# databricks/spark-sklearn

Hardware: NVIDIA H100
Metric: candidate-fits/sec (higher is better)
Workload: dtype f64

## Files before the change

include/b200gs.h:

```cpp
#ifndef B200GS_H
#define B200GS_H

#include <stdint.h>

#ifdef __cplusplus
extern "C" {
#endif

typedef struct gs_handle gs_handle;

enum gs_status {
    GS_OK = 0,
    GS_ERR_CUDA = -1,
    GS_ERR_ARG = -2,
    GS_ERR_NO_DATA = -3,
    GS_ERR_UNSUPPORTED = -4,
    GS_ERR_NUMERIC = -5
};

enum gs_kernel { GS_KERNEL_LINEAR = 0, GS_KERNEL_RBF = 1, GS_KERNEL_POLY = 2, GS_KERNEL_SIGMOID = 3 };
enum gs_dtype { GS_F32 = 0, GS_F64 = 1 };

enum gs_flags {
    GS_RETURN_TRAIN = 1,
// ... 105 lines not shown
    int32_t *test_block, *train_block;
    float *shift;
    float *block_shift;
    double *ystat;
    double *G;
    double *T, *Tw;
    float *A;
    float *rhs;
    double *means;
    float *coef;
    double *qk, *qt;
    double *scores;
    int32_t *n_iter;
    double *gap;
} gs_linear_debug;
int gs_debug_linear(gs_handle *h, int32_t mode, int32_t n_cand, const double *alpha, const double *l1_ratio, int32_t fit_intercept,
                    double tol, int32_t max_iter, int32_t refit, gs_linear_debug *out);

int gs_debug_gemm_nt(gs_handle *h, const float *A, int32_t M, const float *B, int32_t N, int32_t K, float *C);
int gs_debug_gemm_f64(gs_handle *h, const double *A, int32_t M, const double *B, int32_t N, int32_t K, double *C);

double gs_svc_predicted_iterations(int32_t kernel, double C, double gamma, int32_t d);
int32_t gs_svc_cluster_count(const double *cost_desc, int32_t n, int32_t sm_count);
void gs_svc_schedule(const double *cost_desc, int32_t n, int32_t sm_count, int32_t *n_cluster, int32_t *n_exclusive);

typedef struct gs_profile {
    float ms_total;
    float ms_h2d;
    float ms_gram;
    float ms_kernel_matrix;
    float ms_solve;
    float ms_score;
    int64_t launches;
    int64_t smo_iterations;
    double solve_bytes;
    double gram_flops;
    double gram_bytes;
    int64_t h2d_bytes;
    int64_t d2h_bytes;
    float ms_tensor;
    double tensor_flops;
} gs_profile;
int gs_get_profile(const gs_handle *h, gs_profile *out);

#ifdef __cplusplus
}
// ... 3 lines not shown
```

spark_sklearn_b200/csrc/api.cu:

```cuda
#include "common.cuh"
#include <algorithm>
#include <cmath>
#include <cstring>
#include <cstdio>
#include <cstdlib>
#include <map>
#include <numeric>

static std::string g_create_error;

double gs_score_from_counts(int kind, int pos_class, int n_classes, const int *cnt)
{
    auto sup = [&](int c) { return (double)cnt[c * 3 + 0]; };
    auto tp = [&](int c) { return (double)cnt[c * 3 + 1]; };
    auto prd = [&](int c) { return (double)cnt[c * 3 + 2]; };
    auto f1c = [&](int c) { const double den = sup(c) + prd(c); return den > 0 ? 2.0 * tp(c) / den : 0.0; };
    double n = 0, correct = 0;
    for (int c = 0; c < n_classes; c++) { n += sup(c); correct += tp(c); }
    if (!(n > 0)) return NAN;
    switch (kind) {
    case GS_SCORE_DEFAULT: return correct / n;
    case GS_SCORE_BALANCED_ACCURACY: {
        double s = 0; int k = 0;
        for (int c = 0; c < n_classes; c++) if (sup(c) > 0) { s += tp(c) / sup(c); k++; }
// ... 281 lines not shown
{
    if (kernel != GS_KERNEL_RBF) return C;
    const double gd = gamma * (double)d;
    if (!(gd > 0)) return C;
    return std::min(4.0 + 10.3 * std::pow(C * gd, 0.95), 9.0 + 7.3 / gd);
}

extern "C" int32_t gs_svc_cluster_count(const double *cost_desc, int32_t n, int32_t sm_count)
{
    if (!cost_desc || n < 2 || sm_count < 4) return 0;
    double total = 0;
    for (int q = 0; q < n; q++) total += cost_desc[q];
    const int nmax = std::min(n - 1, sm_count / 4);
    double best = 0, clustered = 0;
    int pick = 0;
    for (int k = 0; k <= nmax; k++) {
        const double f = std::max({(total + clustered) / sm_count, 0.9 * cost_desc[k], k > 0 ? 0.5 * cost_desc[0] : 0.0});
        if (k == 0 || f < 0.97 * best) { best = f; pick = k; }
        clustered += cost_desc[k];
    }
    return pick;
}

extern "C" void gs_svc_schedule(const double *cost_desc, int32_t n, int32_t sm_count, int32_t *n_cluster, int32_t *n_exclusive)
{
    if (n_cluster) *n_cluster = 0;
    if (n_exclusive) *n_exclusive = 0;
    if (!cost_desc || n < 2 || sm_count < 8) return;
    std::vector<double> suffix(n + 1, 0.0);
    for (int q = n - 1; q >= 0; q--) suffix[q] = suffix[q + 1] + cost_desc[q];
    double best = -1;
    int bc = 0, be = 0;
    const int max_cl = std::min(n - 1, sm_count / 4);
    for (int nc = 0; nc <= max_cl; nc++) {
        for (int ne = 0; nc + ne < n && 4 * nc + ne <= sm_count - 8; ne++) {
            const int left = sm_count - 4 * nc - ne;
            double t = std::max(0.50 * suffix[nc + ne] / left, 0.78 * cost_desc[nc + ne]);
            if (nc > 0) t = std::max(t, 0.34 * cost_desc[0]);
            if (ne > 0) t = std::max(t, 0.52 * cost_desc[nc]);
            if (best < 0 || t < 0.97 * best || (t < best && nc + ne <= bc + be)) { best = t; bc = nc; be = ne; }
        }
    }
    if (n_cluster) *n_cluster = bc;
    if (n_exclusive) *n_exclusive = be;
}

static int svc_run(gs_handle *h, int n_cand, const int32_t *kernel, const double *Cv, const double *gamma,
                   double tol, int max_iter, uint32_t flags, bool refit, bool nu,
                   double *test_scores, double *train_scores, int32_t *n_iter, int32_t *n_sv,
                   float *fit_ms, float *score_ms, double *pair_coef, double *rho_out, int32_t *pair_iter)
{
    const char *who = nu ? "gs_nusvc" : "gs_svc";
    if (!h) return GS_ERR_ARG;
    if (h->n == 0) { gs_set_error(h, std::string(who) + ": no dataset (call gs_set_data first)"); return GS_ERR_NO_DATA; }
    if (!h->classification) { gs_set_error(h, std::string(who) + ": dataset has no class labels"); return GS_ERR_ARG; }
    if (h->n_classes < 2 || h->n_classes > 32) { gs_set_error(h, std::string(who) + ": need 2..32 classes"); return GS_ERR_UNSUPPORTED; }
    if (n_cand <= 0 || !kernel || !Cv || !gamma) { gs_set_error(h, std::string(who) + ": bad arguments"); return GS_ERR_ARG; }
    if (!h->sample_w.empty()) {
        gs_set_error(h, std::string(who) + ": sample weights (a C per row) are not supported by the SMO kernels; class weights are (gs_set_class_weight)");
        return GS_ERR_UNSUPPORTED;
    }
    if (h->class_w_sets > 1 && h->class_w_sets != (refit ? 1 : h->n_splits)) {
        gs_set_error(h, std::string(who) + ": gs_set_class_weight was given a weight set per split, but not for this number of splits"); return GS_ERR_ARG;
    }
    GS_CUDA(cudaSetDevice(h->device));
    cudaStream_t st = h->stream;
    const int n = (int)h->n, d = (int)h->d, nc = h->n_classes;
// ... 199 lines not shown
        int max_slots = 0;
        bool lean_ok = lmax < 16383 && !(getenv("B200GS_SMO_LEAN") && atoi(getenv("B200GS_SMO_LEAN")) == 0);
        for (int q = 0; q < np && lean_ok; q++) {
            lean_ok = probs[q].nseg > 0 && probs[q].nslots <= smo_lean_max_slots();
            max_slots = std::max(max_slots, probs[q].nslots);
        }
        auto launch_single = [&](const int *ord, int cnt, cudaStream_t s_, bool exclusive) -> cudaError_t {
            for (int inst = search.fast ? 1 : 0; inst >= 0; inst--) {
                const cudaError_t e = lean_ok ? launch_smo_lean(d_probs, ord, cnt, max_slots, inst == 1, exclusive, s_)
                                              : launch_smo(d_probs, ord, cnt, lmax, inst == 1, (int)ldk, s_, &why);
                if (e != cudaSuccess) return e;
                pf.launches++;
            }
            return cudaSuccess;
        };
        int cl = 0, n_cl = 0, n_ex = 0;
        if (!nu && lmax > 2048) {
            if (np * 8 <= h->sm_count) { cl = 8; n_cl = np; }
            else if (np * 4 <= h->sm_count) { cl = 4; n_cl = np; }
            else if (np * 2 <= h->sm_count) { cl = 2; n_cl = np; }
            else {
                std::vector<double> sorted_cost(np);
                for (int q = 0; q < np; q++) sorted_cost[q] = cost[order[q]];
                if (lean_ok) gs_svc_schedule(sorted_cost.data(), np, h->sm_count, &n_cl, &n_ex);
                else n_cl = gs_svc_cluster_count(sorted_cost.data(), np, h->sm_count);
                if (n_cl > 0) cl = 4;
            }
        }
        if (const char *e = getenv("B200GS_SMO_CLUSTER")) { cl = atoi(e); if (n_cl == 0) n_cl = std::max(1, np * 6 / 100); }
        if (const char *e = getenv("B200GS_SMO_CLUSTER_N")) n_cl = std::min(np, atoi(e));
        if (!(cl == 2 || cl == 4 || cl == 8) || lmax > smo_colown_max_rows(cl) || lmax <= 2048) n_cl = 0;
        n_ex = std::max(0, std::min(n_ex, np - n_cl));
        if (nu) {
            for (int inst = search.fast ? 1 : 0; inst >= 0; inst--) {
                const cudaError_t ce = launch_smo_nu(d_probs, nullptr, d_nu, d_order, np, lmax, inst == 1, st, &why);
                if (ce != cudaSuccess) { gs_set_error(h, why.empty() ? std::string("launch_smo_nu: ") + cudaGetErrorString(ce) : why); return why.empty() ? GS_ERR_CUDA : GS_ERR_UNSUPPORTED; }
                pf.launches++;
            }
        } else if (n_cl > 0 || n_ex > 0) {
            cudaEvent_t ready = h->evp.get();
            cudaEventRecord(ready, st);
            cudaError_t ce = cudaSuccess;
            if (n_cl > 0) {
                for (int inst = search.fast ? 1 : 0; inst >= 0 && ce == cudaSuccess; inst--) {
                    ce = launch_smo_colown(d_probs, d_order, n_cl, lmax, cl, inst == 1, st);
                    pf.launches++;
                }
                if (ce != cudaSuccess) { gs_set_error(h, std::string("launch_smo_colown: ") + cudaGetErrorString(ce)); return GS_ERR_CUDA; }
            }
// ... 60 lines not shown
        for (int q = 0; q < np; q++) {
            const int t = prob_task[q];
            task_iter[t] += info[(size_t)q * 4]; task_sv[t] += info[(size_t)q * 4 + 2];
            task_fit_ms[t] += (double)(ns[(size_t)q * 12 + 1] - ns[(size_t)q * 12]) * 1e-6;
            total_iter += info[(size_t)q * 4];
            solve_bytes += (double)info[(size_t)q * 4] * 2.0 * probs[q].l * 4.0;
            if (!std::isfinite(rho[q])) { if (refit) { gs_set_error(h, std::string(who) + "_refit: non-finite intercept"); return GS_ERR_NUMERIC; } task_bad[t] = 1; }
        }
        if (getenv("B200GS_SMO_TIMELINE") && atoi(getenv("B200GS_SMO_TIMELINE"))) {
            unsigned long long t0 = ~0ull;
            for (int q = 0; q < np; q++) if (ns[(size_t)q * 12]) t0 = std::min(t0, ns[(size_t)q * 12]);
            auto span = [&](int a, int b, const char *name) {
                if (b <= a) return;
                double s0 = 1e30, s1 = 0, e0 = 1e30, e1 = 0; long long it_max = 0;
                for (int i = a; i < b; i++) {
                    const int q = order[i];
                    const double st_ = (double)(ns[(size_t)q * 12] - t0) * 1e-6, en = (double)(ns[(size_t)q * 12 + 1] - t0) * 1e-6;
                    s0 = std::min(s0, st_); s1 = std::max(s1, st_); e0 = std::min(e0, en); e1 = std::max(e1, en);
                    it_max = std::max<long long>(it_max, info[(size_t)q * 4]);
                }
                fprintf(stderr, "[timeline] %-9s %4d problems: starts %.2f..%.2f ms, ends %.2f..%.2f ms, longest %lld iterations\n",
                        name, b - a, s0, s1, e0, e1, it_max);
            };
            span(0, n_cl, "cluster"); span(n_cl, n_cl + n_ex, "exclusive"); span(n_cl + n_ex, np, "shared");
            for (int i = 0; i < std::min(np, 16); i++) {
                const int q = order[i];
                fprintf(stderr, "[timeline]   #%d: %d iterations, %.2f -> %.2f ms (%.3f us/iteration)\n", i, info[(size_t)q * 4],
                        (double)(ns[(size_t)q * 12] - t0) * 1e-6, (double)(ns[(size_t)q * 12 + 1] - t0) * 1e-6,
                        (double)(ns[(size_t)q * 12 + 1] - ns[(size_t)q * 12]) * 1e-3 / std::max(1, info[(size_t)q * 4]));
            }
        }
        if (getenv("B200GS_SMO_PROF") && atoi(getenv("B200GS_SMO_PROF"))) {
            int qmax = 0;
            for (int q = 1; q < np; q++) if (info[(size_t)q * 4] > info[(size_t)qmax * 4]) qmax = q;
            const unsigned long long *pn = &ns[(size_t)qmax * 12];
            const double it = (double)info[(size_t)qmax * 4];
            fprintf(stderr, "[smo prof] longest problem: %d iters, %.1f ms (%.2f us/iter); cycles/iter by slot:", info[(size_t)qmax * 4],
                    (double)(pn[1] - pn[0]) * 1e-6, (double)(pn[1] - pn[0]) * 1e-3 / it);
            for (int e = 0; e < 10; e++) fprintf(stderr, " %.0f", pn[2 + e] / it);
            fprintf(stderr, "\n");
        }
        for (size_t v = 0; v < vtasks.size(); v++)
            for (int e = 0; e < 4; e++) all_counts[(size_t)vtask_id[v] * 4 + e] = counts[v * 4 + e];
        if (!refit && h->score_kind == GS_SCORE_ROC_AUC) {
            for (size_t v = 0; v < vtasks.size(); v++) {
                const int k = vtasks[v].fold;
                double na_te = 0, nb_te = 0, na_tr = 0, nb_tr = 0;
                for (int r = 0; r < n; r++) {
                    const bool b = r >= h->class_start[1];
                    if (h->is_test(r, k)) (b ? nb_te : na_te) += 1;
                    else if (h->is_train(r, k)) (b ? nb_tr : na_tr) += 1;
                }
                const unsigned long long *a = &score_raw[v * 4];
                task_score[(size_t)vtask_id[v] * 2 + 0] = na_te * nb_te > 0 ? ((double)a[0] + 0.5 * (double)a[1]) / (na_te * nb_te) : NAN;
                task_score[(size_t)vtask_id[v] * 2 + 1] = na_tr * nb_tr > 0 ? ((double)a[2] + 0.5 * (double)a[3]) / (na_tr * nb_tr) : NAN;
            }
        } else if (!refit && h->score_kind != GS_SCORE_DEFAULT) {
            for (size_t v = 0; v < vtasks.size(); v++)
                for (int sp = 0; sp < 2; sp++)
                    task_score[(size_t)vtask_id[v] * 2 + sp] =
                        gs_score_from_counts(h->score_kind, h->score_pos, nc, &class_counts[(v * 2 + sp) * nc * 3]);
        }
        if (refit) {
// ... 252 lines not shown
```

spark_sklearn_b200/csrc/smo_lean.cu:

```cuda
#include "smo_common.cuh"
#include <algorithm>
#include <type_traits>

namespace {

using namespace smo;

constexpr unsigned LF_UP = 4u, LF_LOW = 8u;
constexpr int POS_SHIFT = 18, SLOT_SHIFT = 4;
constexpr unsigned SLOT_MASK = 0x3fffu;
constexpr unsigned PF_INERT = 0xfffffff0u;

__device__ __forceinline__ unsigned lean_flags(bool ypos, int st)
{
    const bool up = ypos ? st != ST_UPPER : st != ST_LOWER;
    const bool low = ypos ? st != ST_LOWER : st != ST_UPPER;
    return (unsigned)st | (up ? LF_UP : 0u) | (low ? LF_LOW : 0u);
}

template <int N, int I = 0, class F>
__device__ __forceinline__ void lean_loop(F &&f)
{
    if constexpr (I < N) { f(std::integral_constant<int, I>{}); lean_loop<N, I + 1>(f); }
}
// ... 52 lines not shown
                 "mad.wide.u32 wi, %4, 0x20000000, 0x3800000000000000;\n\t"
                 "mad.wide.u32 wj, %5, 0x20000000, 0x3800000000000000;\n\t"
                 "mov.b64 fi, wi;\n\t"
                 "mov.b64 fj, wj;\n\t"
                 "mul.rn.f64 fi, fi, %6;\n\t"
                 "mul.rn.f64 fj, fj, %7;\n\t"
                 "add.rn.f64 fi, fi, fj;\n\t"
                 "add.rn.f64 %0, %0, fi;\n\t"
                 "and.b32 t, %8, %9;\n\t"
                 "setp.ne.u32 pu, t, 0;\n\t"
                 "setp.gt.and.f64 pb, %0, %1, pu;\n\t"
                 "setp.eq.and.f64 pe, %0, %1, pu;\n\t"
                 "selp.f64 %1, %0, %1, pb;\n\t"
                 "selp.b32 %2, %10, %2, pb;\n\t"
                 "selp.b32 %3, 1, %3, pe;\n\t"
                 "}"
                 : "+d"(m), "+d"(la), "+r"(la_k), "+r"(tie)
                 : "r"(__float_as_uint(kvi)), "r"(__float_as_uint(kvj)), "d"(a), "d"(b), "r"(fm), "n"(1u << (2 * K)), "n"(K));
}

struct LeanRed {
    unsigned a_hi[32], a_lo[32], a_pf[32];
    unsigned b_k1[32], b_pf[32], b_k2[32], b_fl[32];
    float b_kq[32]; double b_al[32], b_mg[32];
    double al_i;
    double bc_d[4]; int bc_i[2];
    unsigned x_hi[32], x_lo[32], x_pf[32];
    float x_kq[32]; double x_al[32], x_mg[32];
    double dm[32], dm2[32]; int cnt[32];
    int seg_slot[5], seg_col[4];
    int ysplit;
};

template <int NT, int G, bool FAST, bool PROF>
__global__ void __launch_bounds__(NT, (NT * G >= 4096 || NT >= 1024 ? 1 : 2048 / (NT * G / 2) > 8 ? 8 : 2048 / (NT * G / 2)))
smo_lean_kernel(const SmoProblem *__restrict__ probs, const int *__restrict__ order)
{
    extern __shared__ __align__(16) unsigned char smem_raw[];
    __shared__ LeanRed red;
    constexpr int NW = NT / 32;
    constexpr int KPT = G * 4;
    constexpr int LCAP = NT * KPT;

    const SmoProblem *__restrict__ Pp = probs + order[blockIdx.x];
    if (Pp->guard != nullptr && (*Pp->guard != 0) == FAST) return;
    const int tid = threadIdx.x, lane = tid & 31, warp = tid >> 5;
    const int l = Pp->l;
    const int nslots = Pp->nslots;
    double *const mG = reinterpret_cast<double *>(smem_raw);
    unsigned *const pfS = reinterpret_cast<unsigned *>(mG + LCAP);
    double *const alpha_g = Pp->alpha;
    double *const gbar_g = Pp->Gbar;
    int *const scratch = Pp->scratch;
    const float *__restrict__ const K = Pp->K;
    const int64_t ldk = Pp->ldk;
    const double eps = Pp->eps;
    const double Cc = Pp->C, Cneg = Pp->Cn;
    const bool use_gbar = Pp->shrinking != 0;
    const double *__restrict__ const qd = FAST ? nullptr : Pp->qd;

    unsigned long long t_start = 0;
    if (tid == 0) asm volatile("mov.u64 %0, %%globaltimer;" : "=l"(t_start));

    if (tid == 0) {
        int s = 0;
        for (int e = 0; e < 4; e++) {
            red.seg_slot[e] = e < Pp->nseg ? s : 0x7fffffff;
            red.seg_col[e] = e < Pp->nseg ? Pp->seg_start[e] : 0;
            if (e < Pp->nseg) s += Pp->seg_len[e];
        }
        red.seg_slot[4] = 0x7fffffff;
    }
    __syncthreads();
    auto slot_col = [&](int slot) -> int {
        const int e = (slot >= red.seg_slot[1]) + (slot >= red.seg_slot[2]) + (slot >= red.seg_slot[3]);
        return red.seg_col[e] + (slot - red.seg_slot[e]);
    };
    int gcol[G];
#pragma unroll
    for (int g = 0; g < G; g++) {
        const int s4 = (g * NT + tid) * 4;
        gcol[g] = s4 < nslots ? slot_col(s4) : 0;
    }

    auto m_at = [&](int slot) -> double & { return mG[((slot >> 1) & 1) * (LCAP / 2) + (slot >> 2) * 2 + (slot & 1)]; };
    auto load_m4 = [&](int s4, double (&mv)[4]) {
        const double2 a = *reinterpret_cast<const double2 *>(mG + (s4 >> 1)), b = *reinterpret_cast<const double2 *>(mG + LCAP / 2 + (s4 >> 1));
        mv[0] = a.x; mv[1] = a.y; mv[2] = b.x; mv[3] = b.y;
    };
    auto store_m4 = [&](int s4, const double (&mv)[4]) {
        *reinterpret_cast<double2 *>(mG + (s4 >> 1)) = make_double2(mv[0], mv[1]);
        *reinterpret_cast<double2 *>(mG + LCAP / 2 + (s4 >> 1)) = make_double2(mv[2], mv[3]);
    };
    auto load_pf4 = [&](int s4, unsigned (&pv)[4]) {
        const uint4 p = *reinterpret_cast<const uint4 *>(pfS + s4);
        pv[0] = p.x; pv[1] = p.y; pv[2] = p.z; pv[3] = p.w;
    };

    {
        const int n_pos = Pp->n_pos;
        const int *__restrict__ rows = Pp->rows;
        int ysp = 0x7fffffff;
#pragma unroll
        for (int g = 0; g < G; g++) {
#pragma unroll
            for (int q = 0; q < 4; q++) {
                const int s = (g * NT + tid) * 4 + q;
                unsigned w = PF_INERT;
                double mv = 0.0;
                if (s < nslots) {
                    const int c = gcol[g] + q;
                    int lo = 0, hi = l;
                    while (lo < hi) { const int mid = (lo + hi) >> 1; if (rows[mid] < c) lo = mid + 1; else hi = mid; }
                    if (lo < l && rows[lo] == c) {
                        const bool yp = lo < n_pos;
                        w = ((unsigned)lo << POS_SHIFT) | ((unsigned)s << SLOT_SHIFT) | lean_flags(yp, ST_LOWER);
                        mv = yp ? 1.0 : -1.0;
                        if (lo == n_pos) ysp = s;
                    }
                    alpha_g[s] = 0.0;
                    if (use_gbar) gbar_g[s] = 0.0;
                }
                m_at(s) = mv; pfS[s] = w;
            }
        }
        if (ysp != 0x7fffffff) red.ysplit = ysp;
    }
    __syncthreads();
    const int ysplit = red.ysplit;

    int active = l, iter = 0, timed_out = 0;
    int counter = (l < 1000 ? l : 1000) + 1;
    bool unshrink = false;
    const int max_iter = Pp->max_iter == -1 ? SAFETY_MAX_ITER : Pp->max_iter;
// ... 4 lines not shown
        if constexpr (PROF) {
            const long long now = clock64();
            prof[slot] += now - tprev;
            tprev = now;
        }
    };

    auto QDc = [&](int c) -> double {
        if constexpr (FAST) return 1.0;
        else return qd ? qd[c] : 1.0;
    };
    auto widen = [&](float x) -> double {
        if constexpr (FAST) {
            const unsigned long long r = (unsigned long long)__float_as_uint(x) * 0x20000000ull + 0x3800000000000000ull;
            return __longlong_as_double((long long)r);
        } else return f2d(x);
    };
    auto load_row = [&](int col, float (&kv)[KPT]) {
        const float *__restrict__ Kr = K + (size_t)col * ldk;
#pragma unroll
        for (int g = 0; g < G; g++) {
            float4 v;
            asm volatile("ld.global.nc.L1::no_allocate.v4.f32 {%0, %1, %2, %3}, [%4];"
                         : "=f"(v.x), "=f"(v.y), "=f"(v.z), "=f"(v.w) : "l"(Kr + gcol[g]));
            kv[g * 4 + 0] = v.x; kv[g * 4 + 1] = v.y; kv[g * 4 + 2] = v.z; kv[g * 4 + 3] = v.w;
        }
    };

    double la = -CUDART_INF;
    unsigned la_pf = 0u;
    unsigned fm = 0u;
    static_assert(G <= 4, "the flag mask holds 16 slots");
    auto slot_of = [&](int k) -> int { return ((k >> 2) * NT + tid) * 4 + (k & 3); };
    auto scan_exact = [&](double mv, unsigned w) {
        const bool better = ((w & LF_UP) != 0u) & ((mv > la) | ((mv == la) & (w > la_pf)));
        la = better ? mv : la;
        la_pf = better ? w : la_pf;
    };
    auto local_scan = [&]() {
        la = -CUDART_INF; la_pf = 0u;
#pragma unroll
        for (int g = 0; g < G; g++) {
            const int s4 = (g * NT + tid) * 4;
            double mv[4]; unsigned pv[4];
            load_m4(s4, mv); load_pf4(s4, pv);
#pragma unroll
            for (int q = 0; q < 4; q++) scan_exact(mv[q], pv[q]);
// ... 39 lines not shown
            const int t = base + tid;
            const int sl = t < active ? __ldcg(slot_by_pos + t) : -1;
            int tot;
            const int r = block_rank<NT>(sl >= 0, red.cnt, tot);
            if (sl >= 0) lists[nf + r] = sl;
            nf += tot;
        }
        __syncthreads();
#pragma unroll 1
        for (int g = 0; g < G; g++) {
            const int s4 = (g * NT + tid) * 4;
            unsigned pv[4];
            load_pf4(s4, pv);
            bool in[4];
            double gacc[4];
            bool any = false;
#pragma unroll
            for (int q = 0; q < 4; q++) {
                in[q] = pv[q] >= act_lim && pv[q] < PF_INERT;
                any = any || in[q];
                gacc[q] = in[q] ? __dadd_rn(__ldcg(gbar_g + s4 + q), s4 + q < ysplit ? 1.0 : -1.0) : 0.0;
            }
            if (!any) continue;
            const int gc = gcol[g];
#pragma unroll 4
            for (int r = 0; r < nf; r++) {
                const int fs = __ldcg(lists + r);
                const double av = __ldcg(alpha_g + fs);
                const double af = fs < ysplit ? -av : av;
                const float4 v = __ldg(reinterpret_cast<const float4 *>(K + (size_t)slot_col(fs) * ldk + gc));
                const float kv[4] = {v.x, v.y, v.z, v.w};
#pragma unroll
                for (int q = 0; q < 4; q++)
                    if (in[q]) gacc[q] = __dadd_rn(gacc[q], __dmul_rn(af, widen(kv[q])));
            }
#pragma unroll
            for (int q = 0; q < 4; q++)
                if (in[q]) m_at(s4 + q) = gacc[q];
        }
        __syncthreads();
    };

    unsigned pi = 0u, pj = 0u;
    int col_i = 0, col_j = 0;
    double gmax = 0, mg_j = 0, k_ij = 0, alpha_i = 0, alpha_j = 0;
    float kvi[KPT];
    auto select = [&]() -> bool {
        {
            const unsigned long long key = dkey(la);
            const UArg w = warp_argmax_u((unsigned)(key >> 32), (unsigned)key, la_pf);
            if (lane == 0) { red.a_hi[warp] = w.hi; red.a_lo[warp] = w.lo; red.a_pf[warp] = w.idx; }
            tick(0);
            __syncthreads();
            tick(1);
            const bool v = lane < NW;
            const UArg a = warp_argmax_u(v ? red.a_hi[lane] : 0u, v ? red.a_lo[lane] : 0u, v ? red.a_pf[lane] : 0u);
            pi = a.idx;
            gmax = dkey_inv(((unsigned long long)a.hi << 32) | a.lo);
        }
        if (pi == 0u) return true;
        const int slot_i = (int)((pi >> SLOT_SHIFT) & SLOT_MASK);
        col_i = slot_col(slot_i);
        load_row(col_i, kvi);
        if (tid == 0) red.al_i = __ldcg(alpha_g + slot_i);
        const double QDi = QDc(col_i);
        constexpr unsigned BAND = FAST ? 64u : 514u;
        constexpr unsigned KEY_TINY = 0x0D800000u;
        const float epsf = __double2float_rn(eps);
        auto approx_key = [&](double gd, float gdf, float kvf, int c) -> unsigned {
            if constexpr (FAST) {
// ... 13 lines not shown
        int k1 = 0;
        float kq1 = 0.f;
        float gmxf = 0.f;
        double mvb[4];
        if constexpr (FAST) {
            lean_loop<G * 4>([&](auto kc) {
                constexpr int k = decltype(kc)::value, g = k >> 2, q = k & 3;
                if constexpr (q == 0) load_m4((g * NT + tid) * 4, mvb);
                lean_phase_b_slot<k>(gmax, mvb[q], fm, kvi[k], b1k, b2k, k1, kq1, gmxf);
            });
        } else {
#pragma unroll
            for (int g = 0; g < G; g++) {
                const int s4 = (g * NT + tid) * 4;
                double mv[4];
                load_m4(s4, mv);
#pragma unroll
                for (int q = 0; q < 4; q++) {
                    const int k = g * 4 + q;
                    const double gd = __dsub_rn(gmax, mv[q]);
                    const bool cand = ((fm & (2u << (2 * k))) != 0u) & (gd > 0);
                    const float gdf = cand ? __double2float_rn(gd) : 0.f;
                    gmxf = fmaxf(gmxf, gdf);
                    const unsigned key = cand ? approx_key(gd, gdf, kvi[k], gcol[g] + q) : 0u;
                    const bool gt = key > b1k;
                    b2k = max(b2k, min(b1k, key));
                    b1k = max(b1k, key);
                    k1 = gt ? k : k1;
                    kq1 = gt ? kvi[k] : kq1;
                }
            }
        }
        const unsigned idx1 = b1k ? pfS[slot_of(k1)] : 0u;
        unsigned top1k, top2k;
        {
            const unsigned w1 = __reduce_max_sync(0xffffffffu, b1k);
            const unsigned widx = __reduce_max_sync(0xffffffffu, (b1k == w1) ? idx1 : 0u);
            const unsigned w2 = __reduce_max_sync(0xffffffffu, (idx1 == widx) ? b2k : b1k);
            if (idx1 == widx && widx != 0u) {
                red.b_kq[warp] = kq1;
                red.b_al[warp] = __ldcg(alpha_g + slot_of(k1));
                red.b_mg[warp] = m_at(slot_of(k1));
            }
            const unsigned fb = __reduce_or_sync(0xffffffffu, (gmxf > epsf ? 1u : 0u) | (gmxf == epsf ? 2u : 0u) | (gmxf > 0.f ? 4u : 0u));
            if (lane == 0) { red.b_k1[warp] = w1; red.b_pf[warp] = widx; red.b_k2[warp] = w2; red.b_fl[warp] = fb; }
            tick(2);
            __syncthreads();
            tick(3);
            const bool v = lane < NW;
            const unsigned bk = v ? red.b_k1[lane] : 0u;
            const unsigned bi = v ? red.b_pf[lane] : 0u;
            const unsigned fl = __reduce_or_sync(0xffffffffu, v ? red.b_fl[lane] : 0u);
            top1k = __reduce_max_sync(0xffffffffu, bk);
            pj = __reduce_max_sync(0xffffffffu, (bk == top1k) ? bi : 0u);
            top2k = __reduce_max_sync(0xffffffffu, (v && bi == pj) ? red.b_k2[lane] : bk);
            {
                const int wl = __ffs(__ballot_sync(0xffffffffu, v && bi == pj && pj != 0u)) - 1;
                if (wl >= 0) { k_ij = widen(red.b_kq[wl]); alpha_j = red.b_al[wl]; mg_j = red.b_mg[wl]; }
            }
            if (!(fl & 4u)) return true;
            if (!(fl & 1u)) {
                if (!(fl & 2u)) return true;
                bool viol = false;
#pragma unroll
                for (int g = 0; g < G; g++) {
                    const int s4 = (g * NT + tid) * 4;
                    double mv[4];
                    load_m4(s4, mv);
#pragma unroll
                    for (int q = 0; q < 4; q++) viol = viol | (((fm & (2u << (2 * (g * 4 + q)))) != 0u) & (__dsub_rn(gmax, mv[q]) >= eps));
                }
                if (!__syncthreads_or(viol ? 1 : 0)) return true;
            }
        }
        if (top1k - top2k <= BAND || top1k <= KEY_TINY) {
            if constexpr (PROF) prof[7] += 1;
            const unsigned thrk = (top1k > BAND && top1k > KEY_TINY) ? top1k - BAND : 0u;
            double bestn = -CUDART_INF;
            unsigned bidx = 0u;
            float kqb = 0.f;
#pragma unroll
            for (int g = 0; g < G; g++) {
                const int s4 = (g * NT + tid) * 4;
                double mv[4]; unsigned pv[4];
                load_m4(s4, mv); load_pf4(s4, pv);
#pragma unroll
                for (int q = 0; q < 4; q++) {
                    const double gd = __dsub_rn(gmax, mv[q]);
                    if ((pv[q] & LF_LOW) && gd > 0) {
                        if (approx_key(gd, __double2float_rn(gd), kvi[g * 4 + q], gcol[g] + q) >= thrk) {
                            const double quad = __dsub_rn(__dadd_rn(QDi, QDc(gcol[g] + q)), __dmul_rn(2.0, widen(kvi[g * 4 + q])));
                            const double g2 = __dmul_rn(gd, gd);
                            const double nod = quad > 0 ? __ddiv_rn(g2, quad) : __ddiv_rn(g2, TAU);
                            if (nod > bestn || (nod == bestn && pv[q] > bidx)) { bestn = nod; bidx = pv[q]; kqb = kvi[g * 4 + q]; }
                        }
                    }
                }
            }
            const unsigned long long key = dkey(bestn);
            const UArg w = warp_argmax_u((unsigned)(key >> 32), (unsigned)key, bidx);
            if (bidx == w.idx && w.idx != 0u) {
                red.x_kq[warp] = kqb;
                red.x_al[warp] = __ldcg(alpha_g + (int)((bidx >> SLOT_SHIFT) & SLOT_MASK));
                red.x_mg[warp] = m_at((int)((bidx >> SLOT_SHIFT) & SLOT_MASK));
            }
            if (lane == 0) { red.x_hi[warp] = w.hi; red.x_lo[warp] = w.lo; red.x_pf[warp] = w.idx; }
            __syncthreads();
            const bool v = lane < NW;
            const unsigned xi = v ? red.x_pf[lane] : 0u;
            const UArg b = warp_argmax_u(v ? red.x_hi[lane] : 0u, v ? red.x_lo[lane] : 0u, xi);
            pj = b.idx;
            const int wl = __ffs(__ballot_sync(0xffffffffu, v && xi == pj)) - 1;
            k_ij = widen(red.x_kq[wl]); alpha_j = red.x_al[wl]; mg_j = red.x_mg[wl];
        }
        const int slot_j = (int)((pj >> SLOT_SHIFT) & SLOT_MASK);
        col_j = slot_col(slot_j);
        alpha_i = red.al_i;
        return false;
    };

    auto do_shrink = [&]() {
        double g1 = -CUDART_INF, g2 = -CUDART_INF;
#pragma unroll
        for (int g = 0; g < G; g++) {
            const int s4 = (g * NT + tid) * 4;
            double mv[4]; unsigned pv[4];
            load_m4(s4, mv); load_pf4(s4, pv);
#pragma unroll
            for (int q = 0; q < 4; q++) {
                if (pv[q] & LF_UP) g1 = fmax(g1, mv[q]);
                if (pv[q] & LF_LOW) g2 = fmax(g2, -mv[q]);
            }
        }
        g1 = block_max<NT>(g1, red.dm);
        g2 = block_max<NT>(g2, red.dm2);
        if (!unshrink && __dadd_rn(g1, g2) <= __dmul_rn(eps, 10.0)) {
            unshrink = true;
            rebuild_gradient();
            active = l;
            refresh_flags();
// ... 100 lines not shown
        }
        if (!scan_valid) local_scan();
        if (select()) {
            if (second) break;
            rebuild_gradient();
            active = l;
            refresh_flags();
            __syncthreads();
            scan_valid = false;
            second = true;
            continue;
        }
        if (second) { counter = 1; second = false; }
        ++iter;

        const int slot_i = (int)((pi >> SLOT_SHIFT) & SLOT_MASK), slot_j = (int)((pj >> SLOT_SHIFT) & SLOT_MASK);
        float kvj[KPT];
        load_row(col_j, kvj);
        double a = 0, b = 0, ai_new = 0, aj_new = 0;
        int sti = 0, stj = 0;
        const bool yi = slot_i < ysplit, yj = slot_j < ysplit;
        if (warp == 0) {
            const double Ci = yi ? Cc : Cneg, Cj = yj ? Cc : Cneg;
            const double Gi = yi ? -gmax : gmax;
            const double Gj = yj ? -mg_j : mg_j;
            const double QDi = QDc(col_i), QDj = QDc(col_j);
            const double Qij = (yi == yj) ? k_ij : -k_ij;
            double ai = alpha_i, aj = alpha_j;
            if (yi != yj) {
                double quad = __dadd_rn(__dadd_rn(QDi, QDj), __dmul_rn(2.0, Qij));
                if (quad <= 0) quad = TAU;
                const double delta = __ddiv_rn(__dsub_rn(-Gi, Gj), quad);
                const double diff = __dsub_rn(ai, aj);
                ai = __dadd_rn(ai, delta); aj = __dadd_rn(aj, delta);
                if (diff > 0) { if (aj < 0) { aj = 0; ai = diff; } }
                else          { if (ai < 0) { ai = 0; aj = -diff; } }
                if (diff > __dsub_rn(Ci, Cj)) { if (ai > Ci) { ai = Ci; aj = __dsub_rn(Ci, diff); } }
                else                          { if (aj > Cj) { aj = Cj; ai = __dadd_rn(Cj, diff); } }
            } else {
                double quad = __dsub_rn(__dadd_rn(QDi, QDj), __dmul_rn(2.0, Qij));
                if (quad <= 0) quad = TAU;
                const double delta = __ddiv_rn(__dsub_rn(Gi, Gj), quad);
                const double sum = __dadd_rn(ai, aj);
                ai = __dsub_rn(ai, delta); aj = __dadd_rn(aj, delta);
                if (sum > Ci) { if (ai > Ci) { ai = Ci; aj = __dsub_rn(sum, Ci); } }
                else         { if (aj < 0) { aj = 0; ai = sum; } }
// ... 94 lines not shown
        tick(6);
    }

    __syncthreads();
    if (timed_out && active < l) {
        rebuild_gradient();
        active = l;
    }
    int nsv = 0, nbsv = 0;
    double yg[KPT];
    unsigned wv[KPT];
    {
        double *__restrict__ coef = Pp->coef;
#pragma unroll
        for (int g = 0; g < G; g++) {
            const int s4 = (g * NT + tid) * 4;
            double mv[4]; unsigned pv[4];
            load_m4(s4, mv); load_pf4(s4, pv);
#pragma unroll
            for (int q = 0; q < 4; q++) {
                yg[g * 4 + q] = -mv[q]; wv[g * 4 + q] = pv[q];
                if (pv[q] < PF_INERT) {
                    const double av = __ldcg(alpha_g + s4 + q);
                    coef[gcol[g] + q] = s4 + q < ysplit ? av : -av;
                    nsv += av > 0;
                    nbsv += av >= (s4 + q < ysplit ? Cc : Cneg);
                }
            }
        }
    }
    __syncthreads();
    {
        const unsigned act_lim = (unsigned)active << POS_SHIFT;
#pragma unroll
        for (int k = 0; k < KPT; k++) {
            if (wv[k] < act_lim) {
                const int p = (int)(wv[k] >> POS_SHIFT);
                const int s = ((k >> 2) * NT + tid) * 4 + (k & 3);
                mG[p] = yg[k];
                pfS[p] = (wv[k] & 3u) | (s < ysplit ? 4u : 0u);
            }
        }
    }
    __syncthreads();
    if (tid == 0) {
        int nfree = 0;
        double ub = CUDART_INF, lb = -CUDART_INF, sum = 0;
// ... 10 lines not shown
    for (int s = 16; s; s >>= 1) {
        nsv += __shfl_xor_sync(0xffffffffu, nsv, s);
        nbsv += __shfl_xor_sync(0xffffffffu, nbsv, s);
    }
    if (lane == 0) { red.cnt[warp] = nsv; red.a_pf[warp] = (unsigned)nbsv; }
    __syncthreads();
    if (tid == 0) {
        int s = 0, bs = 0;
        for (int w = 0; w < NW; w++) { s += red.cnt[w]; bs += (int)red.a_pf[w]; }
        int *info = Pp->out_info;
        info[0] = iter; info[1] = timed_out; info[2] = s; info[3] = bs;
        unsigned long long t_end;
        asm volatile("mov.u64 %0, %%globaltimer;" : "=l"(t_end));
        unsigned long long *ns = Pp->out_ns;
        ns[0] = t_start; ns[1] = t_end;
        if constexpr (PROF)
            for (int q = 0; q < 8; q++) ns[2 + q] = (unsigned long long)prof[q];
    }
}

template <int NT, int G, bool FAST, bool PROF>
cudaError_t launch_lean_one(const SmoProblem *probs, const int *order, int n_prob, bool exclusive, cudaStream_t st)
{
    constexpr int LCAP = NT * G * 4;
    const size_t smem = exclusive ? std::max<size_t>((size_t)LCAP * 12, 132 * 1024) : (size_t)LCAP * 12;
    auto kern = smo_lean_kernel<NT, G, FAST, PROF>;
    cudaError_t e = cudaFuncSetAttribute(kern, cudaFuncAttributeMaxDynamicSharedMemorySize, (int)smem);
    if (e != cudaSuccess) return e;
    e = cudaFuncSetAttribute(kern, cudaFuncAttributePreferredSharedMemoryCarveout, cudaSharedmemCarveoutMaxShared);
    if (e != cudaSuccess) return e;
    kern<<<n_prob, NT, smem, st>>>(probs, order);
    return cudaGetLastError();
}

template <int NT, int G>
cudaError_t launch_lean_cfg(const SmoProblem *probs, const int *order, int n_prob, bool fast, bool prof, bool excl, cudaStream_t st)
{
    if (prof) return fast ? launch_lean_one<NT, G, true, true>(probs, order, n_prob, excl, st) : launch_lean_one<NT, G, false, true>(probs, order, n_prob, excl, st);
    return fast ? launch_lean_one<NT, G, true, false>(probs, order, n_prob, excl, st) : launch_lean_one<NT, G, false, false>(probs, order, n_prob, excl, st);
}

}

int smo_lean_max_slots() { return 16384; }

cudaError_t launch_smo_lean(const SmoProblem *d_probs, const int *d_order, int n_prob, int max_slots, bool fast, bool exclusive, cudaStream_t st)
{
    if (n_prob <= 0) return cudaSuccess;
// ... 10 lines not shown
```

spark_sklearn_b200/engine.py:

```python
import ctypes
import os

import numpy as np

_HERE = os.path.dirname(os.path.abspath(__file__))
LIB_PATH = os.path.join(_HERE, "libb200gs.so")

GS_RETURN_TRAIN, GS_GRAM_TENSOR, GS_NO_SHRINKING, GS_TARGET_F32 = 1, 2, 4, 8
KNN_WEIGHTS = {"uniform": 0, "distance": 1}
KNN_METRIC = {"euclidean": 0, "manhattan": 1}
KERNEL_ID = {"linear": 0, "rbf": 1, "poly": 2, "sigmoid": 3}
_PARAM_KERNELS = (2, 3)

_lib = None


class GsProfile(ctypes.Structure):
    _fields_ = [("ms_total", ctypes.c_float), ("ms_h2d", ctypes.c_float), ("ms_gram", ctypes.c_float),
                ("ms_kernel_matrix", ctypes.c_float), ("ms_solve", ctypes.c_float), ("ms_score", ctypes.c_float),
                ("launches", ctypes.c_int64), ("smo_iterations", ctypes.c_int64),
                ("solve_bytes", ctypes.c_double), ("gram_flops", ctypes.c_double), ("gram_bytes", ctypes.c_double),
                ("h2d_bytes", ctypes.c_int64), ("d2h_bytes", ctypes.c_int64),
                ("ms_tensor", ctypes.c_float), ("tensor_flops", ctypes.c_double)]

# ... 55 lines not shown
    L.gs_svr_refit.argtypes = [vp, i32, dbl, dbl, dbl, dbl, i32, u32, vp, vp, vp]
    L.gs_nusvr.argtypes = L.gs_svr.argtypes
    L.gs_nusvr_refit.argtypes = L.gs_svr_refit.argtypes
    L.gs_logreg.argtypes = [vp, i32, vp, dbl, i32, i32, u32, vp, vp, vp, vp, vp]
    L.gs_logreg_refit.argtypes = [vp, dbl, dbl, i32, i32, vp, vp]
    L.gs_linsvc.argtypes = [vp, i32, vp, dbl, i32, i32, dbl, u32, vp, vp, vp, vp, vp]
    L.gs_linsvc_refit.argtypes = [vp, dbl, dbl, i32, i32, dbl, vp, vp]
    L.gs_debug_gemm_f64.argtypes = [vp, vp, i32, vp, i32, i32, vp]
    L.gs_knn.argtypes = [vp, i32, vp, vp, vp, u32, vp, vp, vp, vp]
    L.gs_debug_knn_neighbors.argtypes = [vp, i32, i32, i32, vp, vp]
    L.gs_get_profile.argtypes = [vp, c.POINTER(GsProfile)]
    L.gs_debug_gram.argtypes = [vp, vp, vp]
    L.gs_debug_kernel_matrix.argtypes = [vp, i32, dbl, vp, vp, vp]
    L.gs_debug_decision.argtypes = [vp, i32, dbl, i32, dbl, vp, i32, i32, vp, vp]
    L.gs_debug_score.argtypes = [vp, i32, vp, vp, i32, vp, vp, i32, vp]
    L.gs_debug_gemm_nt.argtypes = [vp, vp, i32, vp, i32, i32, vp]
    L.gs_debug_linear.argtypes = [vp, i32, i32, vp, vp, i32, dbl, i32, i32, vp]
    L.gs_svc_predicted_iterations.argtypes = [i32, dbl, dbl, i32]
    L.gs_svc_predicted_iterations.restype = dbl
    L.gs_svc_cluster_count.argtypes = [vp, i32, i32]
    L.gs_svc_cluster_count.restype = i32
    L.gs_svc_schedule.argtypes = [vp, i32, i32, vp, vp]
    L.gs_svc_schedule.restype = None
    for f in ("gs_create", "gs_set_data", "gs_svc", "gs_svc_refit", "gs_ridge", "gs_ridge_refit", "gs_enet", "gs_enet_refit", "gs_set_targets_f64",
              "gs_svr", "gs_svr_refit", "gs_nusvc", "gs_nusvc_refit", "gs_nusvr", "gs_nusvr_refit", "gs_logreg",
              "gs_logreg_refit", "gs_linsvc", "gs_linsvc_refit", "gs_get_profile", "gs_debug_gram", "gs_debug_kernel_matrix",
              "gs_debug_decision", "gs_debug_score", "gs_debug_linear", "gs_debug_gemm_nt", "gs_debug_gemm_f64", "gs_knn", "gs_debug_knn_neighbors"):
        getattr(L, f).restype = c.c_int
    _lib = L
    return L


def _ptr(a):
    return None if a is None else a.ctypes.data_as(ctypes.c_void_p)


_device_count = None


def device_count():
    global _device_count
    if _device_count is None:
        _device_count = int(load_library().gs_device_count())
    return _device_count


# ... 332 lines not shown
```

Measured before the change: 1027.

## Schedule SMO problems over 4- or 8-CTA clusters and trim lean kernel registers

The SVC scheduler now also considers 8-CTA clusters next to 4-CTA ones, with retuned cost coefficients, and returns the chosen cluster size to the launcher. The lean SMO kernel keeps per-thread column indices in shared memory for large NT*G configurations, and it defers reading the j-side kernel value, alpha and gradient from the reduction buffers instead of carrying them in registers. The aim is better balance of long problems across SMs and lower register pressure. The cost is extra shared-memory traffic and a larger dynamic shared allocation for big configurations. The cost model is heuristic and could pick a worse schedule.

```diff
diff --git a/include/b200gs.h b/include/b200gs.h
--- a/include/b200gs.h
+++ b/include/b200gs.h
@@ -151,6 +151,8 @@
 
 double gs_svc_predicted_iterations(int32_t kernel, double C, double gamma, int32_t d);
 int32_t gs_svc_cluster_count(const double *cost_desc, int32_t n, int32_t sm_count);
+void gs_svc_schedule_sized(const double *cost_desc, int32_t n, int32_t sm_count, int32_t *n_cluster, int32_t *n_exclusive,
+                           int32_t *cluster_size);
 void gs_svc_schedule(const double *cost_desc, int32_t n, int32_t sm_count, int32_t *n_cluster, int32_t *n_exclusive);
 
 typedef struct gs_profile {
diff --git a/spark_sklearn_b200/csrc/api.cu b/spark_sklearn_b200/csrc/api.cu
--- a/spark_sklearn_b200/csrc/api.cu
+++ b/spark_sklearn_b200/csrc/api.cu
@@ -327,27 +327,38 @@
     return pick;
 }
 
-extern "C" void gs_svc_schedule(const double *cost_desc, int32_t n, int32_t sm_count, int32_t *n_cluster, int32_t *n_exclusive)
+extern "C" void gs_svc_schedule_sized(const double *cost_desc, int32_t n, int32_t sm_count, int32_t *n_cluster,
+                                      int32_t *n_exclusive, int32_t *cluster_size)
 {
     if (n_cluster) *n_cluster = 0;
     if (n_exclusive) *n_exclusive = 0;
+    if (cluster_size) *cluster_size = 0;
     if (!cost_desc || n < 2 || sm_count < 8) return;
     std::vector<double> suffix(n + 1, 0.0);
     for (int q = n - 1; q >= 0; q--) suffix[q] = suffix[q + 1] + cost_desc[q];
     double best = -1;
-    int bc = 0, be = 0;
-    const int max_cl = std::min(n - 1, sm_count / 4);
-    for (int nc = 0; nc <= max_cl; nc++) {
-        for (int ne = 0; nc + ne < n && 4 * nc + ne <= sm_count - 8; ne++) {
-            const int left = sm_count - 4 * nc - ne;
-            double t = std::max(0.50 * suffix[nc + ne] / left, 0.78 * cost_desc[nc + ne]);
-            if (nc > 0) t = std::max(t, 0.34 * cost_desc[0]);
-            if (ne > 0) t = std::max(t, 0.52 * cost_desc[nc]);
-            if (best < 0 || t < 0.97 * best || (t < best && nc + ne <= bc + be)) { best = t; bc = nc; be = ne; }
+    int bc = 0, be = 0, bs = 0;
+    for (const int cl : {4, 8}) {
+        const double t_cl = cl == 4 ? 0.39 : 0.36;
+        const int max_cl = std::min(n - 1, sm_count / cl);
+        for (int nc = 0; nc <= max_cl; nc++) {
+            for (int ne = 0; nc + ne < n && cl * nc + ne <= sm_count - 8; ne++) {
+                const int left = sm_count - cl * nc - ne;
+                double t = std::max(0.50 * suffix[nc + ne] / left, 0.81 * cost_desc[nc + ne]);
+                if (nc > 0) t = std::max(t, t_cl * cost_desc[0]);
+                if (ne > 0) t = std::max(t, 0.525 * cost_desc[nc]);
+                if (best < 0 || t < 0.97 * best || (t < best && nc + ne <= bc + be)) { best = t; bc = nc; be = ne; bs = nc > 0 ? cl : 0; }
+            }
         }
     }
     if (n_cluster) *n_cluster = bc;
     if (n_exclusive) *n_exclusive = be;
+    if (cluster_size) *cluster_size = bs;
+}
+
+extern "C" void gs_svc_schedule(const double *cost_desc, int32_t n, int32_t sm_count, int32_t *n_cluster, int32_t *n_exclusive)
+{
+    gs_svc_schedule_sized(cost_desc, n, sm_count, n_cluster, n_exclusive, nullptr);
 }
 
 static int svc_run(gs_handle *h, int n_cand, const int32_t *kernel, const double *Cv, const double *gamma,
@@ -593,9 +604,8 @@
             else {
                 std::vector<double> sorted_cost(np);
                 for (int q = 0; q < np; q++) sorted_cost[q] = cost[order[q]];
-                if (lean_ok) gs_svc_schedule(sorted_cost.data(), np, h->sm_count, &n_cl, &n_ex);
-                else n_cl = gs_svc_cluster_count(sorted_cost.data(), np, h->sm_count);
-                if (n_cl > 0) cl = 4;
+                if (lean_ok) gs_svc_schedule_sized(sorted_cost.data(), np, h->sm_count, &n_cl, &n_ex, &cl);
+                else if ((n_cl = gs_svc_cluster_count(sorted_cost.data(), np, h->sm_count)) > 0) cl = 4;
             }
         }
         if (const char *e = getenv("B200GS_SMO_CLUSTER")) { cl = atoi(e); if (n_cl == 0) n_cl = std::max(1, np * 6 / 100); }
@@ -702,6 +712,7 @@
                 fprintf(stderr, "[timeline] %-9s %4d problems: starts %.2f..%.2f ms, ends %.2f..%.2f ms, longest %lld iterations\n",
                         name, b - a, s0, s1, e0, e1, it_max);
             };
+            if (n_cl > 0) fprintf(stderr, "[timeline] %d-CTA clusters\n", cl);
             span(0, n_cl, "cluster"); span(n_cl, n_cl + n_ex, "exclusive"); span(n_cl + n_ex, np, "shared");
             for (int i = 0; i < std::min(np, 16); i++) {
                 const int q = order[i];
@@ -711,14 +722,18 @@
             }
         }
         if (getenv("B200GS_SMO_PROF") && atoi(getenv("B200GS_SMO_PROF"))) {
-            int qmax = 0;
-            for (int q = 1; q < np; q++) if (info[(size_t)q * 4] > info[(size_t)qmax * 4]) qmax = q;
-            const unsigned long long *pn = &ns[(size_t)qmax * 12];
-            const double it = (double)info[(size_t)qmax * 4];
-            fprintf(stderr, "[smo prof] longest problem: %d iters, %.1f ms (%.2f us/iter); cycles/iter by slot:", info[(size_t)qmax * 4],
-                    (double)(pn[1] - pn[0]) * 1e-6, (double)(pn[1] - pn[0]) * 1e-3 / it);
-            for (int e = 0; e < 10; e++) fprintf(stderr, " %.0f", pn[2 + e] / it);
-            fprintf(stderr, "\n");
+            auto tier = [&](int a, int b, const char *name) {
+                if (b <= a) return;
+                int qmax = order[a];
+                for (int i = a + 1; i < b; i++) if (info[(size_t)order[i] * 4] > info[(size_t)qmax * 4]) qmax = order[i];
+                const unsigned long long *pn = &ns[(size_t)qmax * 12];
+                const double it = (double)std::max(1, info[(size_t)qmax * 4]);
+                fprintf(stderr, "[smo prof] %-9s longest problem: %d iters, %.1f ms (%.3f us/iter); cycles/iter by slot:", name,
+                        info[(size_t)qmax * 4], (double)(pn[1] - pn[0]) * 1e-6, (double)(pn[1] - pn[0]) * 1e-3 / it);
+                for (int e = 0; e < 10; e++) fprintf(stderr, " %.0f", pn[2 + e] / it);
+                fprintf(stderr, "\n");
+            };
+            tier(0, n_cl, "cluster"); tier(n_cl, n_cl + n_ex, "exclusive"); tier(n_cl + n_ex, np, "shared");
         }
         for (size_t v = 0; v < vtasks.size(); v++)
             for (int e = 0; e < 4; e++) all_counts[(size_t)vtask_id[v] * 4 + e] = counts[v * 4 + e];
diff --git a/spark_sklearn_b200/csrc/smo_lean.cu b/spark_sklearn_b200/csrc/smo_lean.cu
--- a/spark_sklearn_b200/csrc/smo_lean.cu
+++ b/spark_sklearn_b200/csrc/smo_lean.cu
@@ -98,15 +98,20 @@
 struct LeanRed {
     unsigned a_hi[32], a_lo[32], a_pf[32];
     unsigned b_k1[32], b_pf[32], b_k2[32], b_fl[32];
-    float b_kq[32]; double b_al[32], b_mg[32];
+    float b_kq[32]; double b_al[32];
     double al_i;
     double bc_d[4]; int bc_i[2];
     unsigned x_hi[32], x_lo[32], x_pf[32];
-    float x_kq[32]; double x_al[32], x_mg[32];
+    float x_kq[32]; double x_al[32];
     double dm[32], dm2[32]; int cnt[32];
     int seg_slot[5], seg_col[4];
     int ysplit;
 };
+
+template <int NT, int G>
+__host__ __device__ constexpr bool lean_gcol_shared() { return NT * G >= 1024; }
+template <int NT, int G>
+constexpr size_t lean_smem_bytes() { return (size_t)NT * G * 4 * 12 + (lean_gcol_shared<NT, G>() ? (size_t)NT * G * 4 : 0); }
 
 template <int NT, int G, bool FAST, bool PROF>
 __global__ void __launch_bounds__(NT, (NT * G >= 4096 || NT >= 1024 ? 1 : 2048 / (NT * G / 2) > 8 ? 8 : 2048 / (NT * G / 2)))
@@ -152,12 +157,20 @@
         const int e = (slot >= red.seg_slot[1]) + (slot >= red.seg_slot[2]) + (slot >= red.seg_slot[3]);
         return red.seg_col[e] + (slot - red.seg_slot[e]);
     };
-    int gcol[G];
+    constexpr bool GCS = lean_gcol_shared<NT, G>();
+    int *const gcolS = reinterpret_cast<int *>(pfS + LCAP);
+    int gcolR[GCS ? 1 : G];
 #pragma unroll
     for (int g = 0; g < G; g++) {
         const int s4 = (g * NT + tid) * 4;
-        gcol[g] = s4 < nslots ? slot_col(s4) : 0;
-    }
+        const int c = s4 < nslots ? slot_col(s4) : 0;
+        if constexpr (GCS) gcolS[g * NT + tid] = c;
+        else gcolR[g] = c;
+    }
+    auto gcol = [&](int g) -> int {
+        if constexpr (GCS) return gcolS[g * NT + tid];
+        else return gcolR[g];
+    };
 
     auto m_at = [&](int slot) -> double & { return mG[((slot >> 1) & 1) * (LCAP / 2) + (slot >> 2) * 2 + (slot & 1)]; };
     auto load_m4 = [&](int s4, double (&mv)[4]) {
@@ -185,7 +198,7 @@
                 unsigned w = PF_INERT;
                 double mv = 0.0;
                 if (s < nslots) {
-                    const int c = gcol[g] + q;
+                    const int c = gcol(g) + q;
                     int lo = 0, hi = l;
                     while (lo < hi) { const int mid = (lo + hi) >> 1; if (rows[mid] < c) lo = mid + 1; else hi = mid; }
                     if (lo < l && rows[lo] == c) {
@@ -236,7 +249,7 @@
         for (int g = 0; g < G; g++) {
             float4 v;
             asm volatile("ld.global.nc.L1::no_allocate.v4.f32 {%0, %1, %2, %3}, [%4];"
-                         : "=f"(v.x), "=f"(v.y), "=f"(v.z), "=f"(v.w) : "l"(Kr + gcol[g]));
+                         : "=f"(v.x), "=f"(v.y), "=f"(v.z), "=f"(v.w) : "l"(Kr + gcol(g)));
             kv[g * 4 + 0] = v.x; kv[g * 4 + 1] = v.y; kv[g * 4 + 2] = v.z; kv[g * 4 + 3] = v.w;
         }
     };
@@ -322,7 +335,7 @@
                 gacc[q] = in[q] ? __dadd_rn(__ldcg(gbar_g + s4 + q), s4 + q < ysplit ? 1.0 : -1.0) : 0.0;
             }
             if (!any) continue;
-            const int gc = gcol[g];
+            const int gc = gcol(g);
 #pragma unroll 4
             for (int r = 0; r < nf; r++) {
                 const int fs = __ldcg(lists + r);
@@ -343,9 +356,10 @@
 
     unsigned pi = 0u, pj = 0u;
     int col_i = 0, col_j = 0;
-    double gmax = 0, mg_j = 0, k_ij = 0, alpha_i = 0, alpha_j = 0;
+    int selw = 0;
     float kvi[KPT];
     auto select = [&]() -> bool {
+        double gmax;
         {
             const unsigned long long key = dkey(la);
             const UArg w = warp_argmax_u((unsigned)(key >> 32), (unsigned)key, la_pf);
@@ -405,7 +419,7 @@
                     const bool cand = ((fm & (2u << (2 * k))) != 0u) & (gd > 0);
                     const float gdf = cand ? __double2float_rn(gd) : 0.f;
                     gmxf = fmaxf(gmxf, gdf);
-                    const unsigned key = cand ? approx_key(gd, gdf, kvi[k], gcol[g] + q) : 0u;
+                    const unsigned key = cand ? approx_key(gd, gdf, kvi[k], gcol(g) + q) : 0u;
                     const bool gt = key > b1k;
                     b2k = max(b2k, min(b1k, key));
                     b1k = max(b1k, key);
@@ -423,7 +437,6 @@
             if (idx1 == widx && widx != 0u) {
                 red.b_kq[warp] = kq1;
                 red.b_al[warp] = __ldcg(alpha_g + slot_of(k1));
-                red.b_mg[warp] = m_at(slot_of(k1));
             }
             const unsigned fb = __reduce_or_sync(0xffffffffu, (gmxf > epsf ? 1u : 0u) | (gmxf == epsf ? 2u : 0u) | (gmxf > 0.f ? 4u : 0u));
             if (lane == 0) { red.b_k1[warp] = w1; red.b_pf[warp] = widx; red.b_k2[warp] = w2; red.b_fl[warp] = fb; }
@@ -439,7 +452,7 @@
             top2k = __reduce_max_sync(0xffffffffu, (v && bi == pj) ? red.b_k2[lane] : bk);
             {
                 const int wl = __ffs(__ballot_sync(0xffffffffu, v && bi == pj && pj != 0u)) - 1;
-                if (wl >= 0) { k_ij = widen(red.b_kq[wl]); alpha_j = red.b_al[wl]; mg_j = red.b_mg[wl]; }
+                selw = wl;
             }
             if (!(fl & 4u)) return true;
             if (!(fl & 1u)) {
@@ -471,8 +484,8 @@
                 for (int q = 0; q < 4; q++) {
                     const double gd = __dsub_rn(gmax, mv[q]);
                     if ((pv[q] & LF_LOW) && gd > 0) {
-                        if (approx_key(gd, __double2float_rn(gd), kvi[g * 4 + q], gcol[g] + q) >= thrk) {
-                            const double quad = __dsub_rn(__dadd_rn(QDi, QDc(gcol[g] + q)), __dmul_rn(2.0, widen(kvi[g * 4 + q])));
+                        if (approx_key(gd, __double2float_rn(gd), kvi[g * 4 + q], gcol(g) + q) >= thrk) {
+                            const double quad = __dsub_rn(__dadd_rn(QDi, QDc(gcol(g) + q)), __dmul_rn(2.0, widen(kvi[g * 4 + q])));
                             const double g2 = __dmul_rn(gd, gd);
                             const double nod = quad > 0 ? __ddiv_rn(g2, quad) : __ddiv_rn(g2, TAU);
                             if (nod > bestn || (nod == bestn && pv[q] > bidx)) { bestn = nod; bidx = pv[q]; kqb = kvi[g * 4 + q]; }
@@ -485,7 +498,6 @@
             if (bidx == w.idx && w.idx != 0u) {
                 red.x_kq[warp] = kqb;
                 red.x_al[warp] = __ldcg(alpha_g + (int)((bidx >> SLOT_SHIFT) & SLOT_MASK));
-                red.x_mg[warp] = m_at((int)((bidx >> SLOT_SHIFT) & SLOT_MASK));
             }
             if (lane == 0) { red.x_hi[warp] = w.hi; red.x_lo[warp] = w.lo; red.x_pf[warp] = w.idx; }
             __syncthreads();
@@ -494,11 +506,10 @@
             const UArg b = warp_argmax_u(v ? red.x_hi[lane] : 0u, v ? red.x_lo[lane] : 0u, xi);
             pj = b.idx;
             const int wl = __ffs(__ballot_sync(0xffffffffu, v && xi == pj)) - 1;
-            k_ij = widen(red.x_kq[wl]); alpha_j = red.x_al[wl]; mg_j = red.x_mg[wl];
+            selw = 32 + wl;
         }
         const int slot_j = (int)((pj >> SLOT_SHIFT) & SLOT_MASK);
         col_j = slot_col(slot_j);
-        alpha_i = red.al_i;
         return false;
     };
 
@@ -645,6 +656,10 @@
         const bool yi = slot_i < ysplit, yj = slot_j < ysplit;
         if (warp == 0) {
             const double Ci = yi ? Cc : Cneg, Cj = yj ? Cc : Cneg;
+            const double gmax = m_at(slot_i), mg_j = m_at(slot_j);
+            const bool xw = selw >= 32;
+            const double k_ij = widen(xw ? red.x_kq[selw - 32] : red.b_kq[selw]);
+            const double alpha_i = red.al_i, alpha_j = xw ? red.x_al[selw - 32] : red.b_al[selw];
             const double Gi = yi ? -gmax : gmax;
             const double Gj = yj ? -mg_j : mg_j;
             const double QDi = QDc(col_i), QDj = QDc(col_j);
@@ -785,7 +800,7 @@
                 yg[g * 4 + q] = -mv[q]; wv[g * 4 + q] = pv[q];
                 if (pv[q] < PF_INERT) {
                     const double av = __ldcg(alpha_g + s4 + q);
-                    coef[gcol[g] + q] = s4 + q < ysplit ? av : -av;
+                    coef[gcol(g) + q] = s4 + q < ysplit ? av : -av;
                     nsv += av > 0;
                     nbsv += av >= (s4 + q < ysplit ? Cc : Cneg);
                 }
@@ -842,8 +857,7 @@
 template <int NT, int G, bool FAST, bool PROF>
 cudaError_t launch_lean_one(const SmoProblem *probs, const int *order, int n_prob, bool exclusive, cudaStream_t st)
 {
-    constexpr int LCAP = NT * G * 4;
-    const size_t smem = exclusive ? std::max<size_t>((size_t)LCAP * 12, 132 * 1024) : (size_t)LCAP * 12;
+    const size_t smem = exclusive ? std::max<size_t>(lean_smem_bytes<NT, G>(), 132 * 1024) : lean_smem_bytes<NT, G>();
     auto kern = smo_lean_kernel<NT, G, FAST, PROF>;
     cudaError_t e = cudaFuncSetAttribute(kern, cudaFuncAttributeMaxDynamicSharedMemorySize, (int)smem);
     if (e != cudaSuccess) return e;
diff --git a/spark_sklearn_b200/engine.py b/spark_sklearn_b200/engine.py
--- a/spark_sklearn_b200/engine.py
+++ b/spark_sklearn_b200/engine.py
@@ -101,6 +101,8 @@
     L.gs_svc_cluster_count.restype = i32
     L.gs_svc_schedule.argtypes = [vp, i32, i32, vp, vp]
     L.gs_svc_schedule.restype = None
+    L.gs_svc_schedule_sized.argtypes = [vp, i32, i32, vp, vp, vp]
+    L.gs_svc_schedule_sized.restype = None
     for f in ("gs_create", "gs_set_data", "gs_svc", "gs_svc_refit", "gs_ridge", "gs_ridge_refit", "gs_enet", "gs_enet_refit", "gs_set_targets_f64",
               "gs_svr", "gs_svr_refit", "gs_nusvc", "gs_nusvc_refit", "gs_nusvr", "gs_nusvr_refit", "gs_logreg",
               "gs_logreg_refit", "gs_linsvc", "gs_linsvc_refit", "gs_get_profile", "gs_debug_gram", "gs_debug_kernel_matrix",
```

Measured after the change: 1084, median of 6. 5.6% higher.
